# ohsnyt/bzip2-rust

Measured on AMD Instinct MI355X. Metric: compress MB/s at -9 (900 KB blocks), 1/2/4/8 MI355X; bit-exact vs C bzip2, higher is better.
Workload: dtype u8; 1 GPU; 1024 MiB per GPU synthetic text at -9 (1194 blocks on this rank), BASELINE configs[2]; raw_bytes_total=1073741824, blocks_rank0=1194, compressed_bytes=323302688

## Files before the change

### bzip2-rust_amd/csrc/bzx_bsort.hip

```cpp
#include <hip/hip_runtime.h>
#include "bzx_host.h"
#include "bzx_wg.h"
#include "bzx_pack.h"

#define BS_NT 1024
#define BS_NW (BS_NT / 64)
#ifndef BS_C
#define BS_C 2048
#endif
#define BS_FW (BS_C / 64)
#define BS_ISO (BS_C / 3)
#ifndef BS_ISO_SHIFT
#define BS_ISO_SHIFT 5
#endif
#ifndef BS_BIN1
#define BS_BIN1 15
#endif
#define BS_BIN2 12
#define BS_NBIN1 (1u << BS_BIN1)
#define BS_TAB_WORDS (BS_NBIN1 + (BS_NBIN1 >> 5))
#define BS_MAX_BK 1024
#ifndef BS_MAX_BIG
#define BS_MAX_BIG 512
#endif
// ... 190 lines not shown
    __syncthreads();
    return b_bcast[4] == 0;
}

struct BzxDeepItem {
    uint32_t blk, st, cnt, dbits;
};

__device__ __forceinline__ uint32_t *rank_array(const BzxBatch &B, uint32_t k, uint32_t which)
{
    if (k >= B.rk_blocks) return nullptr;
    return B.isa2 + ((size_t)k * 2 + which) * BZX_MAX_N;
}

__device__ __forceinline__ void emit_giant(const BzxBatch &B, uint32_t blk, uint64_t *rec_a, const uint64_t *rec_b,
                                           uint32_t st, uint32_t cnt, uint32_t depth, uint32_t bits)
{
    const uint32_t tid = threadIdx.x, base = st & 0x7fffffffu;
    const uint64_t *src = ((st >> 31) ? rec_b : rec_a) + base;
    uint32_t *__restrict__ isa0 = rank_array(B, (uint32_t)BZX_SLAB(B, blk), 0), *__restrict__ isa1 = rank_array(B, (uint32_t)BZX_SLAB(B, blk), 1);
    if (tid == 0) b_bcast[7] = isa0 ? atomicAdd(&B.counters[BZX_CTR_GIANT_CNT], 1u) : 0xFFFFFFFFu;
    __syncthreads();
    const uint32_t at = b_bcast[7];
    const bool listed = at < B.deep_cap;
    for (uint32_t i = tid; i < cnt; i += BS_NT) {
        const uint64_t r = src[i];
        rec_a[base + i] = (uint64_t)REC_IDX(r) | (i == 0 ? 1ull << 32 : 0ull);
        if (isa0) isa0[REC_IDX(r)] = isa1[REC_IDX(r)] = base | (listed ? 0u : RK_COARSE);
    }
    if (tid == 0) {
        atomicMin(&B.blk[blk].n_mtf, depth / bits);
        if (listed) {
            BzxDeepItem it;
            it.blk = blk;
            it.st = base;
            it.cnt = cnt;
            it.dbits = 0;
            reinterpret_cast<BzxDeepItem *>(B.deep_list)[(size_t)2 * B.deep_cap + at] = it;
        }
        atomicAdd(&B.blk[blk].n_groups, 1u);
        if ((atomicOr(&B.blk[blk].status, BZX_ST_RESUME) & BZX_ST_RESUME) == 0)
            B.resume_list[atomicAdd(&B.counters[BZX_CTR_RESUME], 1u)] = blk;
    }
    __syncthreads();
}

__device__ __forceinline__ void block_redo(const BzxBatch &B, uint32_t b)
{
    if ((atomicOr(&B.blk[b].status, BZX_ST_REDO) & BZX_ST_REDO) == 0)
        B.redo_list[atomicAdd(&B.counters[BZX_CTR_REDO], 1u)] = b;
}


__device__ bool deep_process(const BzxBatch &B, uint32_t b, uint32_t j_, uint32_t n, uint32_t bits, const uint8_t *__restrict__ P,
                             uint64_t *__restrict__ rec_a, uint64_t *__restrict__ rec_b, uint32_t done, uint32_t flush_from,
                             int push_lvl)
{
    const uint32_t tid = threadIdx.x;
    bool ok = true;
    while (ok) {
        const uint32_t nbig = b_bcast[3];
        __syncthreads();
        if (done >= nbig) break;
        if (push_lvl >= 0 && done >= flush_from) {
            const uint32_t np = nbig - done;
            if (tid == 0) b_bcast[5] = atomicAdd(&B.counters[BZX_CTR_DEEP_CNT + push_lvl], np);
            __syncthreads();
            const uint32_t at = b_bcast[5];
            __syncthreads();
            if (at + np <= B.deep_cap) {
                BzxDeepItem *dl = reinterpret_cast<BzxDeepItem *>(B.deep_list) + (size_t)(push_lvl & 1) * B.deep_cap + at;
                for (uint32_t q = tid; q < np; q += BS_NT) {
                    const uint32_t r = (done + q) % BS_MAX_BIG;
                    BzxDeepItem it;
                    it.blk = b;
                    it.st = b_big[r][0];
                    it.cnt = b_big[r][1];
                    it.dbits = b_big[r][2] | (bits << 16);
                    dl[q] = it;
                }
                __syncthreads();
                break;
            }
            push_lvl = -1;
        }
        const uint32_t st = b_big[done % BS_MAX_BIG][0], cnt = b_big[done % BS_MAX_BIG][1], depth = b_big[done % BS_MAX_BIG][2];
        done++;
        if (tid == 0) b_bcast[6] = atomicAdd(reinterpret_cast<uint32_t *>(&B.blk[b].pack_word), 1u);
        __syncthreads();
        const uint32_t spent = b_bcast[6];
        const uint32_t base = st & 0x7fffffffu, buf = st >> 31;
        const uint64_t *__restrict__ src = (buf ? rec_b : rec_a) + base;
        uint64_t *__restrict__ dst = (buf ? rec_a : rec_b) + base;
        if (depth + BS_BIN2 + 32 >= n * bits) {
            ok = false;
            break;
        }
        if (depth + BS_BIN2 > BS_MAX_DEPTH || spent >= BS_MAX_SPLITS) {
            emit_giant(B, b, rec_a, rec_b, st, cnt, depth, bits);
            continue;
        }
        constexpr uint32_t NB2 = 1u << BS_BIN2;
        for (uint32_t i = tid; i < NB2 + (NB2 >> 5); i += BS_NT) b_tab[i] = 0;
        if (tid == 0) b_bcast[1] = 0;
        if (tid < 3) b_bcast[8 + tid] = 0;
        __syncthreads();
        for (uint32_t i = tid; i < cnt; i += BS_NT) atomicAdd(&TAB((uint32_t)(src[i] >> (64 - BS_BIN2))), 1u);
// ... 96 lines not shown
                for (uint32_t e = 0; e < 4; e++)
                    if (i0 + e < n) atomicAdd(&TAB((uint32_t)((x[u] << (e * bits)) >> (64 - BS_BIN1))), 1u);
            }
        }
        __syncthreads();
        DIAG_STAMP(99);
        uint32_t nbk = form_buckets<(int)BS_NBIN1, true>(n);
        if (nbk) bucket_setup<BS_BIN1>(nbk);
        __syncthreads();
        DIAG_STAMP(100);
        if (nbk == 0) {
            DIAG_COUNT(106, 1);
            if (tid == 0) block_redo(B, b);
            __syncthreads();
            continue;
        }

        {
            constexpr uint32_t SP_TILE = 8192, SP_V = SP_TILE / (BS_NT * 4);
            static_assert(BS_MAX_BK <= BS_NT && BS_TAB_WORDS >= 32768 + BS_MAX_BK, "tile scan: one bucket per lane");
            uint16_t *tab16 = reinterpret_cast<uint16_t *>(b_tab);
            for (uint32_t i = tid; i < BS_NBIN1 / 2; i += BS_NT) {
                uint32_t v = reinterpret_cast<uint32_t *>(b_tab)[i];
                v |= ((uint32_t)b_b0[v & 1023u] << 10) | ((uint32_t)b_b0[(v >> 16) & 1023u] << 26);
                reinterpret_cast<uint32_t *>(b_tab)[i] = v;
            }
            uint64_t *stage = reinterpret_cast<uint64_t *>(b_tab + 16384);
            uint32_t *tcnt0 = b_tab + 32768;
            uint32_t *delta = b_first;
            uint32_t *tcnt1 = tcnt0 + BS_MAX_BK;
            if (tid < nbk) tcnt0[tid] = tcnt1[tid] = 0;
            uint64_t hi[SP_V], lo[SP_V];
            uint32_t pv[SP_V];
            auto load_tile = [&](uint32_t t0) {
#pragma unroll
                for (uint32_t u = 0; u < SP_V; u++) {
                    const uint32_t i0 = t0 + (u * BS_NT + tid) * 4;
                    hi[u] = lo[u] = 0;
                    pv[u] = 0;
                    if (i0 < n) {
                        uint64_t w2[2];
                        __builtin_memcpy(w2, P + ((i0 * bits) >> 3), 16);
                        hi[u] = w2[0];
                        lo[u] = w2[1];
                        if (i0 >= 1 && i0 + 3 <= n) {
                            __builtin_memcpy(&pv[u], T + i0 - 1, 4);
                        } else {
                            const uint32_t nvalid = n - i0 < 4u ? n - i0 : 4u;
                            for (uint32_t e = 0; e < nvalid; e++) pv[u] |= (uint32_t)T[i0 + e ? i0 + e - 1 : n - 1] << (8 * e);
                        }
                    }
                }
            };
            load_tile(0);
            bzx_lds_barrier();
            uint32_t tpar = 0;
            for (uint32_t t0 = 0; t0 < n; t0 += SP_TILE, tpar ^= 1u) {
                uint32_t *tcnt = tpar ? tcnt1 : tcnt0, *tother = tpar ? tcnt0 : tcnt1;
                uint32_t kr[SP_V * 4], key[SP_V * 4], pvc[SP_V];
#pragma unroll
                for (uint32_t u = 0; u < SP_V; u++) {
                    const uint32_t i0 = t0 + (u * BS_NT + tid) * 4;
                    const uint32_t nvalid = i0 < n ? (n - i0 < 4u ? n - i0 : 4u) : 0u;
                    const uint32_t sh0 = (i0 * bits) & 7u;
                    const uint64_t h = __builtin_bswap64(hi[u]), l = __builtin_bswap64(lo[u]);
                    pvc[u] = pv[u];
#pragma unroll
                    for (uint32_t e = 0; e < 4; e++) {
                        kr[u * 4 + e] = 0xFFFFFFFFu;
                        key[u * 4 + e] = 0;
                        if (e < nvalid) {
                            const uint32_t sh = sh0 + e * bits;
                            const uint64_t w = sh ? (h << sh) | (l >> (64u - sh)) : h;
                            const uint32_t kb = tab16[(uint32_t)(w >> (64 - BS_BIN1))], k = kb & 1023u;
                            key[u * 4 + e] = (uint32_t)((w << (kb >> 10)) >> 32);
                            kr[u * 4 + e] = k | (atomicAdd(&tcnt[k], 1u) << 16);
                        }
                    }
                }
                if (t0 + SP_TILE < n) load_tile(t0 + SP_TILE);
                bzx_lds_barrier();
                {
                    const uint32_t c = tid < nbk ? tcnt[tid] : 0u;
                    const uint32_t incl = bzx_wave_incl_sum(c);
                    uint32_t *wtot = b_scratch + tpar * BS_NW;
                    if (bzx_lane() == 63) wtot[bzx_wave()] = incl;
                    bzx_lds_barrier();
                    uint32_t pre = 0;
                    const uint32_t wv = bzx_wave();
#pragma unroll
                    for (uint32_t i = 0; i < BS_NW; i++) pre += i < wv ? wtot[i] : 0u;
                    const uint32_t ex = pre + incl - c;
                    if (tid < nbk) {
                        tcnt[tid] = ex;
                        tother[tid] = 0;
                        delta[tid] = b_start[tid] + b_cur[tid] - ex;
                        b_cur[tid] += c;
                    }
                }
                bzx_lds_barrier();
#pragma unroll
                for (uint32_t u = 0; u < SP_V; u++)
#pragma unroll
                    for (uint32_t e = 0; e < 4; e++)
                        if (kr[u * 4 + e] != 0xFFFFFFFFu) {
                            const uint32_t k = kr[u * 4 + e] & 0xFFFFu, rel = (u * BS_NT + tid) * 4 + e;
                            stage[tcnt[k] + (kr[u * 4 + e] >> 16)] = ((uint64_t)key[u * 4 + e] << 32) | ((uint64_t)k << 21) | ((uint64_t)rel << 8) |
                                                                     (uint64_t)((pvc[u] >> (8 * e)) & 255u);
                        }
                bzx_lds_barrier();
                const uint32_t tn = n - t0 < SP_TILE ? n - t0 : SP_TILE;
#pragma unroll
                for (uint32_t u = 0; u < SP_TILE / BS_NT; u++) {
                    const uint32_t i = u * BS_NT + tid;
                    if (i < tn) {
                        const uint64_t r = stage[i];
                        const uint32_t k = (uint32_t)(r >> 21) & 1023u, rel = (uint32_t)(r >> 8) & 8191u;
                        rec_a[delta[k] + i] = (r & 0xFFFFFFFF00000000ull) | ((uint64_t)(t0 + rel) << 12) | ((r & 255ull) << 4);
                    }
                }
            }
        }
        __syncthreads();
        DIAG_STAMP(101);
        bool ok = bucket_emit<BS_BIN1>(B, b, j_, nbk, 0, 0, 0, bits, 0, 0);
        DIAG_STAMP(102);

        if (ok) ok = deep_process(B, b, j_, n, bits, P, rec_a, rec_b, 0, 0, BZX_DEEP_LEVELS > 0 ? 0 : -1);
        DIAG_STAMP(103);
        if (!ok) DIAG_COUNT(107, 1);
        if (!ok && tid == 0) block_redo(B, b);
        __syncthreads();
    }
    DIAG_FLUSH();
}

__global__ __launch_bounds__(BS_NT) void bzx_bsplit_deep_kernel(BzxBatch B)
{
    const uint32_t tid = threadIdx.x, lvl = B.deep_lvl;
    const uint32_t listed = B.counters[BZX_CTR_DEEP_CNT + lvl];
    const uint32_t n_items = listed < B.deep_cap ? listed : B.deep_cap;
    if (n_items == 0) return;
    DIAG_T0();
    const BzxDeepItem *list = reinterpret_cast<const BzxDeepItem *>(B.deep_list) + (size_t)(lvl & 1u) * B.deep_cap;
    for (;;) {
        if (tid == 0) b_bcast[0] = atomicAdd(&B.counters[BZX_CTR_DEEP_FETCH + lvl], 1u);
        __syncthreads();
        const uint32_t i = b_bcast[0];
        __syncthreads();
        if (i >= n_items) break;
        const BzxDeepItem d = list[i];
        if (d.cnt == 0) continue;
        const uint32_t b = d.blk;
        if (__atomic_load_n(&B.blk[b].status, __ATOMIC_RELAXED) & BZX_ST_REDO) continue;
        const uint32_t n = B.blk[b].n, bits = d.dbits >> 16;
        const size_t sb = BZX_SLAB(B, b);
        const uint8_t *__restrict__ P = B.pk + sb * BZX_PK_STRIDE;
        uint64_t *__restrict__ rec_a = B.rec_a + sb * BZX_MAX_N;
        uint64_t *__restrict__ rec_b = B.rec_b + sb * BZX_MAX_N;
        if (tid == 0) {
            b_bcast[3] = 1;
            b_bcast[4] = 0;
            b_big[0][0] = d.st;
            b_big[0][1] = d.cnt;
            b_big[0][2] = d.dbits & 0xFFFFu;
        }
        __syncthreads();
        const bool ok = deep_process(B, b, (b - B.blk_first) / B.blk_step, n, bits, P, rec_a, rec_b, 0, 1,
                                     lvl + 1 < BZX_DEEP_LEVELS ? (int)lvl + 1 : -1);
        if (!ok && tid == 0) block_redo(B, b);
        __syncthreads();
    }
    DIAG_FLUSH();
}

#ifndef SK_NT
#define SK_NT 256
#endif
#define SK_NW (SK_NT / 64)
#define BS_E (BS_C / SK_NT)
#define SK_DB 8
#define SK_ND (1u << SK_DB)
static_assert(BS_C % SK_NT == 0 && BS_E >= 1 && BS_E <= 8, "bucket capacity");

__shared__ uint64_t s_x[BS_C];
__shared__ __attribute__((aligned(16))) uint64_t s_w[BS_C + 4];
__shared__ __attribute__((aligned(16))) uint32_t s_cnt[SK_NW][SK_ND];
__shared__ uint32_t s_dbase[SK_ND];
__shared__ uint32_t s_part[4];
__shared__ uint64_t s_f[BS_FW + 1];
__shared__ uint32_t s_med[BS_C / BS_TINY + 1];
__shared__ uint32_t s_large[BS_C / BS_MED + 1];
__shared__ uint32_t s_rc[2][4];
__shared__ uint32_t s_bc[8];
__shared__ uint32_t s_m[2];
__shared__ uint32_t s_red[SK_NW][4];

__device__ __forceinline__ uint32_t uni(uint32_t v) { return bzx_uni(v); }
__device__ __forceinline__ uint32_t tid_here() { return bzx_tid_here(); }
__device__ __forceinline__ BzxBucket uni(BzxBucket b)
{
    BzxBucket r;
    r.blk = uni(b.blk);
    r.start = uni(b.start);
    r.cnt = uni(b.cnt);
    if (r.cnt >> 31) r.cnt = 0;
    r.dbits = uni(b.dbits);
    return r;
}

__device__ __forceinline__ void wave_rank(uint32_t *wc, uint32_t d, bool valid, uint32_t lane, uint32_t &old, uint32_t &rank)
{
    uint64_t m = __ballot(valid);
    uint32_t plo = (uint32_t)m, phi = (uint32_t)(m >> 32);
#pragma unroll
    for (int b = 0; b < SK_DB; b++) {
        const uint32_t mask = 0u - ((d >> b) & 1u);
        m = __ballot((d >> b) & 1u);
        plo &= ~((uint32_t)m ^ mask);
        phi &= ~((uint32_t)(m >> 32) ^ mask);
    }
    const uint64_t peers = ((uint64_t)phi << 32) | plo;
    rank = (uint32_t)__popcll(peers & ((1ull << lane) - 1ull));
    old = wc[d];
    lds_order();
    if (valid && rank == 0) atomicAdd(&wc[d], (uint32_t)__popcll(peers));
    lds_order();
}

__device__ __attribute__((noinline)) void wg_radix_sort(uint32_t base, uint32_t cnt, int lo, int hi)
{
    uint64_t *A = s_w + base;
    const uint32_t tid = threadIdx.x, lane = bzx_lane(), wave = bzx_wave();
    const uint32_t rows = (cnt + SK_NT - 1) / SK_NT, chunk = rows * 64;
    if (tid == 0) {
// ... 95 lines not shown
            a1 &= s_red[w][3];
        }
        diff = ((uint64_t)(o1 & ~a1) << 32) | (o0 & ~a0);
    }
    uint32_t *wc = s_cnt[wave];
    uint32_t *wb = reinterpret_cast<uint32_t *>(s_w) + wave * SK_ND;
    for (int shift = lo; shift < hi; shift += SK_DB) {
        if (((diff >> shift) & (uint64_t)(SK_ND - 1)) == 0) continue;
#pragma unroll
        for (uint32_t i = 0; i < SK_ND / 64; i++) wc[i * 64 + lane] = 0;
        lds_order();
        uint64_t v[BS_E];
        uint32_t old[BS_E];
#pragma unroll
        for (uint32_t j = 0; j < BS_E; j++) {
            const uint32_t e = wave * chunk + j * 64 + lane;
            v[j] = j < rows && e < cnt ? A[e] : 0ull;
        }
#pragma unroll
        for (uint32_t j = 0; j < BS_E; j++) {
            const uint32_t e = wave * chunk + j * 64 + lane;
            old[j] = bzx_lds_ticket(&wc[(uint32_t)(v[j] >> shift) & (SK_ND - 1)], j < rows && e < cnt);
        }
        __syncthreads();
        {
            static_assert(SK_ND == 4 * 64, "four digits per lane");
            uint32_t mine[4], tot[4], sum = 0;
#pragma unroll
            for (uint32_t i = 0; i < 4; i++) mine[i] = tot[i] = 0;
#pragma unroll
            for (uint32_t w = 0; w < SK_NW; w++) {
                const uint4 c = *reinterpret_cast<const uint4 *>(&s_cnt[w][4 * lane]);
                const uint32_t cc[4] = {c.x, c.y, c.z, c.w};
#pragma unroll
                for (uint32_t i = 0; i < 4; i++) {
                    if (w < wave) mine[i] += cc[i];
                    tot[i] += cc[i];
                }
            }
#pragma unroll
            for (uint32_t i = 0; i < 4; i++) sum += tot[i];
            uint32_t run = bzx_wave_incl_sum(sum) - sum;
            uint4 o;
            o.x = run + mine[0];
            run += tot[0];
            o.y = run + mine[1];
            run += tot[1];
            o.z = run + mine[2];
            run += tot[2];
            o.w = run + mine[3];
            *reinterpret_cast<uint4 *>(&wb[4 * lane]) = o;
        }
        lds_order();
#pragma unroll
        for (uint32_t j = 0; j < BS_E; j++) {
            const uint32_t e = wave * chunk + j * 64 + lane;
            if (j < rows && e < cnt) A[wb[(uint32_t)(v[j] >> shift) & (SK_ND - 1)] + old[j]] = v[j];
        }
        __syncthreads();
    }
}

template <bool TICKETS>
__device__ __attribute__((noinline)) void wave_radix_sort(uint32_t base, uint32_t s, int lo, int hi)
{
    constexpr uint32_t ROWS = BS_MED / 64;
    uint64_t *A = s_w + base;
    uint32_t *wc = s_cnt[bzx_wave()];
    const uint32_t lane = bzx_lane();
    const uint32_t rows = (s + 63u) / 64u;
    uint64_t v[ROWS];
    uint64_t diff = 0;
    {
        const uint64_t a0 = A[0];
#pragma unroll
        for (uint32_t j = 0; j < ROWS; j++) {
            const uint32_t e = j * 64 + lane;
            v[j] = e < s ? A[e] : 0ull;
            if (e < s) diff |= v[j] ^ a0;
        }
#pragma unroll
        for (int sh = 32; sh > 0; sh >>= 1) diff |= __shfl_xor(diff, sh);
    }
    for (int shift = lo; shift < hi; shift += SK_DB) {
        if (((diff >> shift) & (uint64_t)(SK_ND - 1)) == 0) continue;
#pragma unroll
        for (uint32_t i = 0; i < SK_ND / 64; i++) wc[i * 64 + lane] = 0;
        lds_order();
        uint32_t old[ROWS], rk[ROWS];
#pragma unroll
        for (uint32_t j = 0; j < ROWS; j++) {
            old[j] = rk[j] = 0;
            if (j < rows) {
                if (TICKETS) old[j] = bzx_lds_ticket(&wc[(uint32_t)(v[j] >> shift) & (SK_ND - 1)], j * 64 + lane < s);
                else wave_rank(wc, (uint32_t)(v[j] >> shift) & (SK_ND - 1), j * 64 + lane < s, lane, old[j], rk[j]);
            }
        }
        {
            uint32_t c[SK_ND / 64], sum = 0;
#pragma unroll
            for (uint32_t i = 0; i < SK_ND / 64; i++) {
                c[i] = wc[(SK_ND / 64) * lane + i];
                sum += c[i];
            }
            uint32_t run = bzx_wave_incl_sum(sum) - sum;
            lds_order();
#pragma unroll
            for (uint32_t i = 0; i < SK_ND / 64; i++) {
                wc[(SK_ND / 64) * lane + i] = run;
                run += c[i];
            }
        }
        lds_order();
#pragma unroll
        for (uint32_t j = 0; j < ROWS; j++)
            if (j * 64 + lane < s) A[wc[(uint32_t)(v[j] >> shift) & (SK_ND - 1)] + old[j] + rk[j]] = v[j];
        lds_order();
#pragma unroll
        for (uint32_t j = 0; j < ROWS; j++) {
            const uint32_t e = j * 64 + lane;
            v[j] = e < s ? A[e] : 0ull;
        }
        lds_order();
    }
}

__device__ __forceinline__ uint32_t fbit(uint32_t p) { return (uint32_t)(s_f[p >> 6] >> (p & 63u)) & 1u; }
__device__ __forceinline__ void fset(uint32_t p) { atomicOr((unsigned long long *)&s_f[p >> 6], 1ull << (p & 63u)); }

__device__ __forceinline__ bool tiny_bounds(uint32_t p, uint32_t &gs, uint32_t &ge)
{
    const uint32_t wi = p >> 6, bi = p & 63u;
    uint64_t w = s_f[wi] & (~0ull >> (63u - bi));
    if (w) {
        gs = wi * 64 + 63u - (uint32_t)__builtin_clzll(w);
    } else {
        if (wi == 0) return false;
        w = s_f[wi - 1];
        if (!w) return false;
        gs = (wi - 1) * 64 + 63u - (uint32_t)__builtin_clzll(w);
    }
    w = bi == 63u ? 0ull : s_f[wi] & (~0ull << (bi + 1u));
    if (w) {
        ge = wi * 64 + (uint32_t)__builtin_ctzll(w);
    } else {
        w = s_f[wi + 1];
        if (!w) return false;
        ge = (wi + 1) * 64 + (uint32_t)__builtin_ctzll(w);
    }
    return ge - gs <= BS_TINY;
}

__device__ __forceinline__ void mark_changes(uint32_t base, uint32_t s, int lo, uint32_t t, uint32_t step)
{
    for (uint32_t e = 1 + t; e < s; e += step)
        if ((s_w[base + e] >> lo) != (s_w[base + e - 1] >> lo)) fset(base + e);
}

__device__ __forceinline__ bool any_big(uint32_t base, uint32_t s, uint32_t t, uint32_t step)
{
    bool big = false;
    for (uint32_t e = t; e < s; e += step) {
        uint32_t gs, ge;
        big |= !tiny_bounds(base + e, gs, ge);
    }
    return big;
}

__device__ __forceinline__ void wave_sort_mark(uint32_t base, uint32_t s, int lo, uint32_t lane)
// ... 93 lines not shown
        wg_radix_sort(gs, sz, 48, 64);
        mark_changes(gs, sz, 48, tid, SK_NT);
        if (tid == 0) s_bc[2] = 0;
        __syncthreads();
        if (any_big(gs, sz, tid, SK_NT)) s_bc[2] = 1;
        __syncthreads();
        if (s_bc[2]) {
            wg_radix_sort(gs, sz, 14, 64);
            mark_changes(gs, sz, 14, tid, SK_NT);
        }
    }
    __syncthreads();
}

template <typename RankOf>
__device__ __forceinline__ void rank_tiny_groups(uint32_t amask, uint32_t nrow, const RankOf &rank_of, uint32_t (&dst_)[BS_E],
                                                 uint64_t (&my)[BS_E])
{
#pragma unroll
    for (uint32_t j = 0; j < BS_E; j++) {
        dst_[j] = 0xFFFFFFFFu;
        my[j] = 0;
        uint32_t a_ = 0, sz = 0;
        if ((amask >> j) & 1u) {
            const uint32_t p = rank_of(j);
            uint32_t e_;
            if (tiny_bounds(p, a_, e_) && e_ - a_ > 1) {
                sz = e_ - a_;
                my[j] = s_w[p];
            }
        }
        if (j < nrow) {
            uint32_t r = 0, rk = 0;
            const uint64_t myc = my[j] & ~W_POS_MASK;
            for (uint32_t i = 0; i < sz; i += 4) {
                uint64_t wq[4];
#pragma unroll
                for (uint32_t k = 0; k < 4; k++) wq[k] = s_w[a_ + i + k];
#pragma unroll
                for (uint32_t k = 0; k < 4; k++) {
                    const bool in = i + k < sz;
                    r += in && wq[k] < my[j];
                    rk += in && wq[k] < myc;
                }
            }
            if (sz) dst_[j] = (a_ + r) | (r != rk ? 0u : 0x80000000u);
        }
    }
    __syncthreads();
}

__device__ __forceinline__ void place_ranked(const uint32_t (&dst_)[BS_E], const uint64_t (&my)[BS_E])
{
#pragma unroll
    for (uint32_t j = 0; j < BS_E; j++) {
        if (dst_[j] != 0xFFFFFFFFu) {
            const uint32_t q = dst_[j] & 0x7FFFFFFFu;
            s_w[q] = my[j];
            if ((dst_[j] >> 31) && !fbit(q)) fset(q);
        }
    }
    __syncthreads();
}

#define LIST(which, i) (reinterpret_cast<uint16_t *>(s_x)[4u * (i) + 2u + (which)])

template <bool ALL>
__device__ __attribute__((noinline)) void list_tied(uint32_t n, uint32_t from, uint32_t to)
{
    const uint32_t tid = tid_here(), lane = tid & 63u;
    const uint32_t nrow = (n + SK_NT - 1) / SK_NT;
#pragma unroll
    for (uint32_t j = 0; j < BS_E; j++) {
        if (j < nrow) {
            const uint32_t i = j * SK_NT + tid;
            uint32_t p = 0;
            bool t = false;
            if (i < n) {
                p = ALL ? i : (uint32_t)LIST(from, i);
                t = !(fbit(p) && fbit(p + 1));
            }
            const uint64_t mk = __ballot(t);
            if (mk) {
                uint32_t base = 0;
                if (lane == 0) base = atomicAdd(&s_m[to], (uint32_t)__popcll(mk));
                base = bzx_bcast0(base);
                if (t) LIST(to, base + (uint32_t)__popcll(mk & ((1ull << lane) - 1ull))) = (uint16_t)p;
            }
        }
    }
}

__device__ __forceinline__ bool initial_sort(uint32_t cnt)
{
    const uint32_t tid = tid_here(), lane = tid & 63u, wave = tid >> 6;
    uint64_t fm[BS_E];
    wg_radix_sort_opt(cnt, 64 - BS_KEYBITS, 64);
    int bad = 0;
#pragma unroll
    for (uint32_t j = 0; j < BS_E; j++) {
        const uint32_t p = j * SK_NT + tid;
        s_w[p] = p;
        const uint64_t kp = s_x[p] >> (64 - BS_KEYBITS), kq = p ? s_x[p - 1] >> (64 - BS_KEYBITS) : 0ull;
        const bool f = p >= cnt || p == 0 || kp != kq;
        bad |= p < cnt && p > 0 && kp < kq;
        fm[j] = __ballot(f);
        if (lane == 0) s_f[j * SK_NW + wave] = fm[j];
    }
    if (tid == 0) s_f[BS_FW] = ~0ull;
    if (__syncthreads_or(bad)) return false;
#pragma unroll
    for (uint32_t j = 0; j < BS_E; j++) {
// ... 140 lines not shown
        }
        if (tid < 4) s_rc[0][tid] = 0;
        if (tid < 2) s_m[tid] = 0;
        DIAG_STAMP(65);
        if (!initial_sort(cnt)) {
            if (tid == 0) {
                atomicAdd(&B.counters[BZX_CTR_STAT0 + 15], 1u);
                block_redo(B, b);
            }
            PREFETCH_NEXT();
            __syncthreads();
            it = nit;
            nit = uni(nit2);
            n_cur = uni(n_nx);
            st_cur = uni(st_nx);
            continue;
        }
        DIAG_STAMP(67);

        uint32_t dcur = depth0 + BS_KEYBITS;
        bool fail = false;
        uint32_t lpar = 0;
        __syncthreads();
        DIAG_STAMP(73);
        for (uint32_t round = 0;; round++) {
            tid = tid_here();
            lane = tid & 63u;
            wave = tid >> 6;
            const uint32_t par = round & 1u;
            const uint32_t m = uni(s_m[lpar]);
            if (m == 0) break;
            if (m <= 64) {
                DIAG_COUNT(89, 1);
                if (wave == 0) {
                    dcur = wave_rounds(P, bits, nbits, m, lpar, round, dcur);
                    if (lane == 0) s_bc[3] = dcur;
                }
                __syncthreads();
                dcur = uni(s_bc[3]);
                fail = dcur >> 31;
                dcur &= 0x7FFFFFFFu;
                DIAG_STAMP(70);
                break;
            }
            if (!(round < BS_ROUNDS && dcur < nbits)) {
                DIAG_COUNT(round >= BS_ROUNDS ? 84 : 85, 1);
                fail = true;
                break;
            }
            DIAG_COUNT(80, 1);
            DIAG_COUNT(88, m);
            const uint32_t nrow = (m + SK_NT - 1) / SK_NT;
            uint32_t amask = 0, hmask = 0;
            uint32_t pq[BS_E], xa[BS_E];
#pragma unroll
            for (uint32_t j = 0; j < BS_E; j++) {
                pq[j] = 0;
                xa[j] = 0;
                if (j < nrow) {
                    const uint32_t i = j * SK_NT + tid;
                    if (i < m) {
                        const uint32_t p = LIST(lpar, i);
                        amask |= 1u << j;
                        hmask |= fbit(p) << j;
                        pq[j] = p | ((uint32_t)(s_w[p] & W_POS_MASK) << 16);
                    }
                }
            }
#pragma unroll
            for (uint32_t j = 0; j < BS_E; j++) {
                if ((amask >> j) & 1u) {
                    uint32_t x = REC_IDX(s_x[pq[j] >> 16]) * bits + dcur;
                    if (x >= nbits) x -= nbits;
                    xa[j] = x;
                }
            }
            uint64_t g[BS_E];
#pragma unroll
            for (uint32_t j = 0; j < BS_E; j++) g[j] = ((amask >> j) & 1u) ? pk_window_bit(P, xa[j]) : 0ull;
            const auto rank_of = [&](uint32_t j) { return pq[j] & 0xFFFFu; };
            list_big_groups(hmask, par, rank_of);
#pragma unroll
            for (uint32_t j = 0; j < BS_E; j++)
                if ((amask >> j) & 1u) s_w[pq[j] & 0xFFFFu] = (g[j] & ~W_POS_MASK) | (uint64_t)(pq[j] >> 16);
            if (tid == 0) {
                s_rc[par ^ 1u][0] = s_rc[par ^ 1u][1] = s_rc[par ^ 1u][2] = s_rc[par ^ 1u][3] = 0;
                s_m[lpar ^ 1u] = 0;
            }
            __syncthreads();
            DIAG_STAMP(68);
            const uint32_t nmed = s_rc[par][1], nlarge = s_rc[par][2];
            if (nmed | nlarge) {
                DIAG_COUNT(86, nmed);
                DIAG_COUNT(87, nlarge);
                sort_listed_groups(par, nmed, nlarge, tid, lane);
                DIAG_STAMP(69);
            }
            tid = tid_here();
            lane = tid & 63u;
            wave = tid >> 6;
            uint32_t dst_[BS_E];
            uint64_t my[BS_E];
            rank_tiny_groups(amask, nrow, rank_of, dst_, my);
            DIAG_STAMP(70);
            place_ranked(dst_, my);
            DIAG_STAMP(71);
            list_tied<false>(m, lpar, lpar ^ 1u);
            __syncthreads();
            DIAG_STAMP(73);
            lpar ^= 1u;
            dcur += 50;
        }
        PREFETCH_NEXT();
        tid = tid_here();
        if (fail || B.bsort_mode == 1) {
            uint64_t *__restrict__ sax = B.rec_a + BZX_SLAB(B, b) * BZX_MAX_N + start;
            const uint32_t rk = uni(B.blk[b].n_selectors);
            uint32_t *__restrict__ isa0 = rank_array(B, rk, 0), *__restrict__ isa1 = rank_array(B, rk, 1);
#pragma unroll
            for (uint32_t j = 0; j < BS_E; j++) {
                const uint32_t p = j * SK_NT + tid;
                if (p < cnt) {
                    const uint32_t rot = REC_IDX(s_x[(uint32_t)(s_w[p] & W_POS_MASK)]);
                    const uint32_t f0 = fbit(p);
                    sax[p] = (uint64_t)rot | ((uint64_t)f0 << 32);
                    if (isa0) {
                        const uint32_t head = f0 ? p : group_start(p);
                        isa0[rot] = start + head;
                        if (f0 && fbit(p + 1)) isa1[rot] = start + head;
                    }
                }
            }
            if (fail) {
                uint32_t *__restrict__ cl = reinterpret_cast<uint32_t *>(B.rec_b + BZX_SLAB(B, b) * BZX_MAX_N + start);
                uint64_t mk[BS_E];
                lane = tid & 63u;
                wave = tid >> 6;
#pragma unroll
                for (uint32_t j = 0; j < BS_E; j++) mk[j] = tied_mask(s_f[j * SK_NW + wave], s_f[j * SK_NW + wave + 1]);
                slot_counts_publish(mk, BS_E);
                __syncthreads();
                uint32_t before[BS_E];
                const uint32_t total = slot_counts_sum(BS_E, before);
#pragma unroll
                for (uint32_t j = 0; j < BS_E; j++) {
                    if ((mk[j] >> lane) & 1ull) {
                        const uint32_t p = j * SK_NT + tid;
                        const uint32_t rot = REC_IDX(s_x[(uint32_t)(s_w[p] & W_POS_MASK)]);
                        cl[before[j] + (uint32_t)__popcll(mk[j] & ((1ull << lane) - 1ull))] = p | (fbit(p) << 11) | (rot << 12);
                    }
                }
                if (tid == 0) {
                    atomicMin(&B.blk[b].n_mtf, dcur / bits);
                    B.bk_list[idx].cnt = cnt | 0x80000000u;
                    const uint32_t ri = atomicAdd(&B.counters[BZX_CTR_RK_ITEMS], 1u);
                    B.rk_list[ri] = idx;
                    B.rk_list[B.bk_cap + ri] = total;
                    atomicAdd(&B.counters[BZX_CTR_RK_OPEN], 1u);
                    atomicAdd(&B.blk[b].n_groups, 1u);
                    if ((atomicOr(&B.blk[b].status, BZX_ST_RESUME) & BZX_ST_RESUME) == 0)
                        B.resume_list[atomicAdd(&B.counters[BZX_CTR_RESUME], 1u)] = b;
                }
            }
        }
        {
            constexpr uint32_t OUT_E = 8;
            uint8_t *__restrict__ L = B.bwt + BZX_SLAB(B, b) * BZX_BLK_STRIDE + start;
            const uint32_t p0 = tid * OUT_E;
            if (p0 < cnt) {
                const uint32_t rot = tid >> 2;
                uint32_t pos[OUT_E];
#pragma unroll
                for (uint32_t k = 0; k < OUT_E; k++) pos[k] = (uint32_t)(s_w[p0 + ((k + rot) & (OUT_E - 1))] & W_POS_MASK);
                uint64_t bytes = 0;
#pragma unroll
                for (uint32_t k = 0; k < OUT_E; k++) {
                    const uint32_t kk = (k + rot) & (OUT_E - 1);
                    const uint32_t r = reinterpret_cast<const uint32_t *>(s_x)[2u * pos[k]];
                    bytes |= (uint64_t)REC_PREV(r) << (8 * kk);
                    if (p0 + kk < cnt && REC_IDX(r) == 0) B.blk[b].orig_ptr = start + p0 + kk;
                }
                if (p0 + OUT_E <= cnt) {
                    __builtin_memcpy(L + p0, &bytes, 8);
                } else {
                    for (uint32_t k = 0; p0 + k < cnt; k++) L[p0 + k] = (uint8_t)(bytes >> (8 * k));
                }
            }
            DIAG_COUNT(83, 1);
        }
        __syncthreads();
        DIAG_STAMP(72);
        it = nit;
        nit = uni(nit2);
        n_cur = uni(n_nx);
        st_cur = uni(st_nx);
    }
    DIAG_FLUSH();
}

__global__ __launch_bounds__(SK_NT, SK_WAVES_PER_SIMD) void bzx_bsort_kernel(BzxBatch B) { bsort_body(B); }
__global__ __launch_bounds__(SK_NT, SK_WAVES_PER_SIMD) void bzx_bfill_kernel(BzxBatch B) { bsort_body(B); }

#define RK_CHUNK 16
struct RkMeta {
    uint32_t bi, T, blk, start, cnt, n, rk, h0;
};
__shared__ RkMeta s_meta[RK_CHUNK];

__device__ __forceinline__ uint32_t rk_fetch_chunk(const BzxBatch &B, uint32_t n_items, uint32_t &open)
{
    __shared__ uint32_t s_fetch[2];
    __syncthreads();
    if (threadIdx.x < 64) {
        uint32_t base = 0;
        if (threadIdx.x == 0) base = atomicAdd(&B.counters[B.rk_fetch], (uint32_t)RK_CHUNK);
        base = __shfl(base, 0);
        const uint32_t i = base + threadIdx.x;
        bool op = false;
        if (threadIdx.x < RK_CHUNK && i < n_items) {
            RkMeta m;
            m.bi = B.rk_list[i];
            m.T = B.rk_list[B.bk_cap + i];
            const BzxBucket it = B.bk_list[m.bi];
            op = !(it.dbits >> 31);
            m.blk = it.blk;
            m.start = it.start & 0x7fffffffu;
            m.cnt = it.cnt & 0x7fffffffu;
            m.n = B.blk[it.blk].n;
            m.rk = B.blk[it.blk].n_selectors;
            m.h0 = B.blk[it.blk].n_mtf;
            s_meta[threadIdx.x] = m;
        }
        const uint64_t m = __ballot(op);
        if (threadIdx.x == 0) {
// ... 558 lines not shown
```

### bzip2-rust_amd/csrc/bzx_wg.h

```cpp
#pragma once
#include <hip/hip_runtime.h>
#include <stdint.h>

#define BZX_WAVE 64

#ifdef BZX_HIP_EMU
#define bzx_lds_barrier() __syncthreads()
#else
#define bzx_lds_barrier() asm volatile("s_waitcnt lgkmcnt(0)\n\ts_barrier" ::: "memory")
#endif

#ifdef BZX_HIP_EMU
#define bzx_wave_sync() hipemu::wave_sync()
#else
#define bzx_wave_sync()                                      \
    do {                                                     \
        __builtin_amdgcn_fence(__ATOMIC_SEQ_CST, "wavefront"); \
        __builtin_amdgcn_wave_barrier();                     \
    } while (0)
#endif


#ifdef BZX_HIP_EMU
__device__ inline uint32_t bzx_lds_ticket(uint32_t *ctr, bool valid)
{
    static uintptr_t who[16][64];
    const uint32_t lane = threadIdx.x & 63u, wave = threadIdx.x >> 6;
    const uintptr_t me = valid ? (uintptr_t)ctr : 0;
    who[wave][lane] = me;
    hipemu::wave_sync();
    uint32_t before = 0, same = 0;
    for (uint32_t l = 0; l < 64; l++) {
        if (valid && who[wave][l] == me) {
            same++;
            if (l < lane) before++;
        }
    }
    const uint32_t base = valid ? *ctr : 0u;
    hipemu::wave_sync();
    if (valid && before == 0) *ctr = base + same;
    hipemu::wave_sync();
    return base + before;
}
#else
__device__ __forceinline__ uint32_t bzx_lds_ticket(uint32_t *ctr, bool valid) { return valid ? atomicAdd(ctr, 1u) : 0u; }
#endif
#ifdef BZX_HIP_EMU
#define lds_order() hipemu::wave_sync()
__device__ __forceinline__ uint32_t bzx_uni(uint32_t v) { return v; }
__device__ __forceinline__ uint32_t bzx_bcast0(uint32_t v) { return __shfl(v, 0); }
__device__ __forceinline__ uint32_t bzx_tid_here() { return threadIdx.x; }
#define bzx_drain_stores() do {} while (0)
#else
#define lds_order() asm volatile("" ::: "memory")
__device__ __forceinline__ uint32_t bzx_uni(uint32_t v) { return (uint32_t)__builtin_amdgcn_readfirstlane((int)v); }
__device__ __forceinline__ uint32_t bzx_bcast0(uint32_t v) { return (uint32_t)__builtin_amdgcn_readfirstlane((int)v); }
__device__ __forceinline__ uint32_t bzx_tid_here()
{
    uint32_t t = threadIdx.x;
    asm volatile("" : "+v"(t));
    return t;
}
#define bzx_drain_stores() asm volatile("s_waitcnt vmcnt(0)" ::: "memory")
#endif

#ifdef BZX_HIP_EMU
#define BZX_HOST_PORTABLE 0u
#define BZX_MBUF_CHUNK_MIN ((size_t)64 << 10)
#else
#define BZX_HOST_PORTABLE hipHostMallocPortable
#define BZX_MBUF_CHUNK_MIN ((size_t)16 << 20)
#endif

#ifdef BZX_HIP_EMU
__device__ inline uint32_t bzx_lane_prev(uint32_t v)
{
    const uint32_t y = __shfl_up(v, 1);
    return (threadIdx.x & 63u) ? y : 0u;
}
#else
__device__ __forceinline__ uint32_t bzx_lane_prev(uint32_t v)
{
    return (uint32_t)__builtin_amdgcn_update_dpp(0, (int)v, 0x138, 0xf, 0xf, false);
}
#endif

__device__ __forceinline__ uint32_t bzx_lane() { return threadIdx.x & 63u; }
__device__ __forceinline__ uint32_t bzx_wave() { return threadIdx.x >> 6; }

__device__ __forceinline__ uint64_t bzx_match_any(uint32_t d, int nbits, bool valid)
{
    uint64_t peers = __ballot(valid);
    for (int b = 0; b < nbits; b++) {
        const bool bit = (d >> b) & 1u;
        const uint64_t m = __ballot(bit);
        peers &= bit ? m : ~m;
    }
    return peers;
}

#ifdef BZX_HIP_EMU
#define BZX_DPP_SCAN(v, OP, IDENT)                                           \
    do {                                                                     \
        const uint32_t lane_ = bzx_lane();                                   \
        for (uint32_t d_ = 1; d_ < 64; d_ <<= 1) {                           \
            const uint32_t y_ = __shfl_up(v, d_);                            \
// ... 161 lines not shown
```

Measured before the change: 29650 MB/s.

## Batch LDS loads ahead of dependent stores across bucket-sort kernels

Restructures several hot loops in the block-sort kernels so independent LDS and global loads are issued as a batch before their dependent atomics and stores. It adds a full-tile fast path in the initial split, hoists scatter addresses and flag-word loads, processes the refine loop in groups of up to four rows, and adds an asm register barrier (bzx_landed) to force loads to complete before use. The aim is more memory-level parallelism and fewer serialized LDS round trips. In exchange it raises register pressure, which can lower occupancy, and duplicates code paths.

```diff
diff --git a/bzip2-rust_amd/csrc/bzx_bsort.hip b/bzip2-rust_amd/csrc/bzx_bsort.hip
--- a/bzip2-rust_amd/csrc/bzx_bsort.hip
+++ b/bzip2-rust_amd/csrc/bzx_bsort.hip
@@ -266,7 +266,7 @@
 }
 
 
-__device__ bool deep_process(const BzxBatch &B, uint32_t b, uint32_t j_, uint32_t n, uint32_t bits, const uint8_t *__restrict__ P,
+__device__ __forceinline__ bool deep_process(const BzxBatch &B, uint32_t b, uint32_t j_, uint32_t n, uint32_t bits, const uint8_t *__restrict__ P,
                              uint64_t *__restrict__ rec_a, uint64_t *__restrict__ rec_b, uint32_t done, uint32_t flush_from,
                              int push_lvl)
 {
@@ -469,12 +469,48 @@
                     }
                 }
             };
+            auto window_landed = [&]() {
+#pragma unroll
+                for (uint32_t u = 0; u < SP_V; u++) {
+                    bzx_landed(hi[u]);
+                    bzx_landed(lo[u]);
+                    bzx_landed(pv[u]);
+                }
+            };
             load_tile(0);
+            window_landed();
             bzx_lds_barrier();
             uint32_t tpar = 0;
-            for (uint32_t t0 = 0; t0 < n; t0 += SP_TILE, tpar ^= 1u) {
+            const uint32_t ns = bzx_uni(n);
+            for (uint32_t t0 = 0; t0 < ns; t0 += SP_TILE, tpar ^= 1u) {
                 uint32_t *tcnt = tpar ? tcnt1 : tcnt0, *tother = tpar ? tcnt0 : tcnt1;
                 uint32_t kr[SP_V * 4], key[SP_V * 4], pvc[SP_V];
+                const bool full = t0 + SP_TILE <= ns;
+                if (full) {
+                    uint64_t w[SP_V * 4];
+                    uint32_t kb[SP_V * 4];
+#pragma unroll
+                    for (uint32_t u = 0; u < SP_V; u++) {
+                        const uint32_t i0 = t0 + (u * BS_NT + tid) * 4;
+                        const uint32_t sh0 = (i0 * bits) & 7u;
+                        const uint64_t h = __builtin_bswap64(hi[u]), l = __builtin_bswap64(lo[u]);
+                        pvc[u] = pv[u];
+#pragma unroll
+                        for (uint32_t e = 0; e < 4; e++) {
+                            const uint32_t sh = sh0 + e * bits;
+                            w[u * 4 + e] = sh ? (h << sh) | (l >> (64u - sh)) : h;
+                        }
+                    }
+#pragma unroll
+                    for (uint32_t q = 0; q < SP_V * 4; q++) kb[q] = tab16[(uint32_t)(w[q] >> (64 - BS_BIN1))];
+#pragma unroll
+                    for (uint32_t q = 0; q < SP_V * 4; q++) kr[q] = atomicAdd(&tcnt[kb[q] & 1023u], 1u);
+#pragma unroll
+                    for (uint32_t q = 0; q < SP_V * 4; q++) {
+                        key[q] = (uint32_t)((w[q] << (kb[q] >> 10)) >> 32);
+                        kr[q] = (kb[q] & 1023u) | (kr[q] << 16);
+                    }
+                } else {
 #pragma unroll
                 for (uint32_t u = 0; u < SP_V; u++) {
                     const uint32_t i0 = t0 + (u * BS_NT + tid) * 4;
@@ -495,6 +531,7 @@
                         }
                     }
                 }
+                }
                 if (t0 + SP_TILE < n) load_tile(t0 + SP_TILE);
                 bzx_lds_barrier();
                 {
@@ -516,6 +553,19 @@
                     }
                 }
                 bzx_lds_barrier();
+                if (full) {
+                    uint32_t tb[SP_V * 4];
+#pragma unroll
+                    for (uint32_t q = 0; q < SP_V * 4; q++) tb[q] = tcnt[kr[q] & 0xFFFFu];
+#pragma unroll
+                    for (uint32_t u = 0; u < SP_V; u++)
+#pragma unroll
+                        for (uint32_t e = 0; e < 4; e++) {
+                            const uint32_t q = u * 4 + e, k = kr[q] & 0xFFFFu, rel = (u * BS_NT + tid) * 4 + e;
+                            stage[tb[q] + (kr[q] >> 16)] = ((uint64_t)key[q] << 32) | ((uint64_t)k << 21) | ((uint64_t)rel << 8) |
+                                                           (uint64_t)((pvc[u] >> (8 * e)) & 255u);
+                        }
+                } else {
 #pragma unroll
                 for (uint32_t u = 0; u < SP_V; u++)
 #pragma unroll
@@ -525,8 +575,23 @@
                             stage[tcnt[k] + (kr[u * 4 + e] >> 16)] = ((uint64_t)key[u * 4 + e] << 32) | ((uint64_t)k << 21) | ((uint64_t)rel << 8) |
                                                                      (uint64_t)((pvc[u] >> (8 * e)) & 255u);
                         }
+                }
                 bzx_lds_barrier();
+                window_landed();
                 const uint32_t tn = n - t0 < SP_TILE ? n - t0 : SP_TILE;
+                if (full) {
+                    uint64_t r[SP_TILE / BS_NT];
+                    uint32_t dl[SP_TILE / BS_NT];
+#pragma unroll
+                    for (uint32_t u = 0; u < SP_TILE / BS_NT; u++) r[u] = stage[u * BS_NT + tid];
+#pragma unroll
+                    for (uint32_t u = 0; u < SP_TILE / BS_NT; u++) dl[u] = delta[(uint32_t)(r[u] >> 21) & 1023u];
+#pragma unroll
+                    for (uint32_t u = 0; u < SP_TILE / BS_NT; u++) {
+                        const uint32_t rel = (uint32_t)(r[u] >> 8) & 8191u;
+                        rec_a[dl[u] + u * BS_NT + tid] = (r[u] & 0xFFFFFFFF00000000ull) | ((uint64_t)(t0 + rel) << 12) | ((r[u] & 255ull) << 4);
+                    }
+                } else {
 #pragma unroll
                 for (uint32_t u = 0; u < SP_TILE / BS_NT; u++) {
                     const uint32_t i = u * BS_NT + tid;
@@ -535,6 +600,7 @@
                         const uint32_t k = (uint32_t)(r >> 21) & 1023u, rel = (uint32_t)(r >> 8) & 8191u;
                         rec_a[delta[k] + i] = (r & 0xFFFFFFFF00000000ull) | ((uint64_t)(t0 + rel) << 12) | ((r & 255ull) << 4);
                     }
+                }
                 }
             }
         }
@@ -598,6 +664,7 @@
 #define BS_E (BS_C / SK_NT)
 #define SK_DB 8
 #define SK_ND (1u << SK_DB)
+#define BS_G (BS_E < 4 ? BS_E : 4)
 static_assert(BS_C % SK_NT == 0 && BS_E >= 1 && BS_E <= 8, "bucket capacity");
 
 __shared__ uint64_t s_x[BS_C];
@@ -799,10 +866,15 @@
             *reinterpret_cast<uint4 *>(&wb[4 * lane]) = o;
         }
         lds_order();
+        uint32_t at[BS_E];
+#pragma unroll
+        for (uint32_t j = 0; j < BS_E; j++) at[j] = wb[(uint32_t)(v[j] >> shift) & (SK_ND - 1)] + old[j];
+#pragma unroll
+        for (uint32_t j = 0; j < BS_E; j++) bzx_landed(at[j]);
 #pragma unroll
         for (uint32_t j = 0; j < BS_E; j++) {
             const uint32_t e = wave * chunk + j * 64 + lane;
-            if (j < rows && e < cnt) A[wb[(uint32_t)(v[j] >> shift) & (SK_ND - 1)] + old[j]] = v[j];
+            if (j < rows && e < cnt) A[at[j]] = v[j];
         }
         __syncthreads();
     }
@@ -838,10 +910,8 @@
 #pragma unroll
         for (uint32_t j = 0; j < ROWS; j++) {
             old[j] = rk[j] = 0;
-            if (j < rows) {
-                if (TICKETS) old[j] = bzx_lds_ticket(&wc[(uint32_t)(v[j] >> shift) & (SK_ND - 1)], j * 64 + lane < s);
-                else wave_rank(wc, (uint32_t)(v[j] >> shift) & (SK_ND - 1), j * 64 + lane < s, lane, old[j], rk[j]);
-            }
+            if (TICKETS) old[j] = bzx_lds_ticket(&wc[(uint32_t)(v[j] >> shift) & (SK_ND - 1)], j * 64 + lane < s);
+            else if (j < rows) wave_rank(wc, (uint32_t)(v[j] >> shift) & (SK_ND - 1), j * 64 + lane < s, lane, old[j], rk[j]);
         }
         {
             uint32_t c[SK_ND / 64], sum = 0;
@@ -859,9 +929,14 @@
             }
         }
         lds_order();
+        uint32_t at[ROWS];
+#pragma unroll
+        for (uint32_t j = 0; j < ROWS; j++) at[j] = wc[(uint32_t)(v[j] >> shift) & (SK_ND - 1)] + old[j] + rk[j];
+#pragma unroll
+        for (uint32_t j = 0; j < ROWS; j++) bzx_landed(at[j]);
 #pragma unroll
         for (uint32_t j = 0; j < ROWS; j++)
-            if (j * 64 + lane < s) A[wc[(uint32_t)(v[j] >> shift) & (SK_ND - 1)] + old[j] + rk[j]] = v[j];
+            if (j * 64 + lane < s) A[at[j]] = v[j];
         lds_order();
 #pragma unroll
         for (uint32_t j = 0; j < ROWS; j++) {
@@ -1061,12 +1136,15 @@
 
 __device__ __forceinline__ void place_ranked(const uint32_t (&dst_)[BS_E], const uint64_t (&my)[BS_E])
 {
+    uint64_t fw[BS_E];
+#pragma unroll
+    for (uint32_t j = 0; j < BS_E; j++) fw[j] = s_f[dst_[j] != 0xFFFFFFFFu ? (dst_[j] & 0x7FFFFFFFu) >> 6 : 0u];
 #pragma unroll
     for (uint32_t j = 0; j < BS_E; j++) {
         if (dst_[j] != 0xFFFFFFFFu) {
             const uint32_t q = dst_[j] & 0x7FFFFFFFu;
             s_w[q] = my[j];
-            if ((dst_[j] >> 31) && !fbit(q)) fset(q);
+            if ((dst_[j] >> 31) && !((fw[j] >> (q & 63u)) & 1ull)) fset(q);
         }
     }
     __syncthreads();
@@ -1313,37 +1391,48 @@
             DIAG_COUNT(88, m);
             const uint32_t nrow = (m + SK_NT - 1) / SK_NT;
             uint32_t amask = 0, hmask = 0;
-            uint32_t pq[BS_E], xa[BS_E];
-#pragma unroll
-            for (uint32_t j = 0; j < BS_E; j++) {
-                pq[j] = 0;
-                xa[j] = 0;
-                if (j < nrow) {
-                    const uint32_t i = j * SK_NT + tid;
-                    if (i < m) {
-                        const uint32_t p = LIST(lpar, i);
-                        amask |= 1u << j;
-                        hmask |= fbit(p) << j;
-                        pq[j] = p | ((uint32_t)(s_w[p] & W_POS_MASK) << 16);
-                    }
-                }
-            }
-#pragma unroll
-            for (uint32_t j = 0; j < BS_E; j++) {
-                if ((amask >> j) & 1u) {
-                    uint32_t x = REC_IDX(s_x[pq[j] >> 16]) * bits + dcur;
+            uint32_t pq[BS_E];
+            const auto rank_of = [&](uint32_t j) { return pq[j] & 0xFFFFu; };
+#pragma unroll
+            for (uint32_t j = 0; j < BS_E; j++) pq[j] = 0;
+#pragma unroll
+            for (uint32_t h0 = 0; h0 < BS_E; h0 += BS_G) {
+                if (h0 >= nrow) break;
+                uint32_t fl[BS_G], xa[BS_G];
+#pragma unroll
+                for (uint32_t k = 0; k < BS_G; k++) {
+                    const uint32_t j = h0 + k, i = j * SK_NT + tid;
+                    const bool has = j < nrow && i < m;
+                    amask |= (uint32_t)has << j;
+                    pq[j] = LIST(lpar, has ? i : 0u);
+                }
+#pragma unroll
+                for (uint32_t k = 0; k < BS_G; k++) {
+                    fl[k] = reinterpret_cast<const uint32_t *>(s_f)[pq[h0 + k] >> 5];
+                    xa[k] = reinterpret_cast<const uint32_t *>(s_w)[2u * pq[h0 + k]];
+                }
+#pragma unroll
+                for (uint32_t k = 0; k < BS_G; k++) {
+                    const uint32_t j = h0 + k;
+                    hmask |= (((fl[k] >> (pq[j] & 31u)) & 1u) & (amask >> j)) << j;
+                    pq[j] |= (xa[k] & (uint32_t)W_POS_MASK) << 16;
+                }
+#pragma unroll
+                for (uint32_t k = 0; k < BS_G; k++) xa[k] = reinterpret_cast<const uint32_t *>(s_x)[2u * (pq[h0 + k] >> 16)];
+#pragma unroll
+                for (uint32_t k = 0; k < BS_G; k++) {
+                    uint32_t x = REC_IDX(xa[k]) * bits + dcur;
                     if (x >= nbits) x -= nbits;
-                    xa[j] = x;
-                }
-            }
-            uint64_t g[BS_E];
-#pragma unroll
-            for (uint32_t j = 0; j < BS_E; j++) g[j] = ((amask >> j) & 1u) ? pk_window_bit(P, xa[j]) : 0ull;
-            const auto rank_of = [&](uint32_t j) { return pq[j] & 0xFFFFu; };
-            list_big_groups(hmask, par, rank_of);
-#pragma unroll
-            for (uint32_t j = 0; j < BS_E; j++)
-                if ((amask >> j) & 1u) s_w[pq[j] & 0xFFFFu] = (g[j] & ~W_POS_MASK) | (uint64_t)(pq[j] >> 16);
+                    xa[k] = ((amask >> (h0 + k)) & 1u) ? x : 0u;
+                }
+                uint64_t g[BS_G];
+#pragma unroll
+                for (uint32_t k = 0; k < BS_G; k++) g[k] = pk_window_bit(P, xa[k]);
+                list_big_groups(hmask & (((1u << BS_G) - 1u) << h0), par, rank_of);
+#pragma unroll
+                for (uint32_t k = 0; k < BS_G; k++)
+                    if ((amask >> (h0 + k)) & 1u) s_w[pq[h0 + k] & 0xFFFFu] = (g[k] & ~W_POS_MASK) | (uint64_t)(pq[h0 + k] >> 16);
+            }
             if (tid == 0) {
                 s_rc[par ^ 1u][0] = s_rc[par ^ 1u][1] = s_rc[par ^ 1u][2] = s_rc[par ^ 1u][3] = 0;
                 s_m[lpar ^ 1u] = 0;
@@ -1433,14 +1522,18 @@
                 uint32_t pos[OUT_E];
 #pragma unroll
                 for (uint32_t k = 0; k < OUT_E; k++) pos[k] = (uint32_t)(s_w[p0 + ((k + rot) & (OUT_E - 1))] & W_POS_MASK);
+                uint32_t r[OUT_E];
+#pragma unroll
+                for (uint32_t k = 0; k < OUT_E; k++) r[k] = reinterpret_cast<const uint32_t *>(s_x)[2u * pos[k]];
                 uint64_t bytes = 0;
+                uint32_t row0 = 0xFFFFFFFFu;
 #pragma unroll
                 for (uint32_t k = 0; k < OUT_E; k++) {
                     const uint32_t kk = (k + rot) & (OUT_E - 1);
-                    const uint32_t r = reinterpret_cast<const uint32_t *>(s_x)[2u * pos[k]];
-                    bytes |= (uint64_t)REC_PREV(r) << (8 * kk);
-                    if (p0 + kk < cnt && REC_IDX(r) == 0) B.blk[b].orig_ptr = start + p0 + kk;
-                }
+                    bytes |= (uint64_t)REC_PREV(r[k]) << (8 * kk);
+                    if (p0 + kk < cnt && REC_IDX(r[k]) == 0) row0 = start + p0 + kk;
+                }
+                if (row0 != 0xFFFFFFFFu) B.blk[b].orig_ptr = row0;
                 if (p0 + OUT_E <= cnt) {
                     __builtin_memcpy(L + p0, &bytes, 8);
                 } else {
diff --git a/bzip2-rust_amd/csrc/bzx_wg.h b/bzip2-rust_amd/csrc/bzx_wg.h
--- a/bzip2-rust_amd/csrc/bzx_wg.h
+++ b/bzip2-rust_amd/csrc/bzx_wg.h
@@ -51,7 +51,9 @@
 __device__ __forceinline__ uint32_t bzx_bcast0(uint32_t v) { return __shfl(v, 0); }
 __device__ __forceinline__ uint32_t bzx_tid_here() { return threadIdx.x; }
 #define bzx_drain_stores() do {} while (0)
-#else
+#define bzx_landed(x) do {} while (0)
+#else
+#define bzx_landed(x) asm volatile("" : "+v"(x))
 #define lds_order() asm volatile("" ::: "memory")
 __device__ __forceinline__ uint32_t bzx_uni(uint32_t v) { return (uint32_t)__builtin_amdgcn_readfirstlane((int)v); }
 __device__ __forceinline__ uint32_t bzx_bcast0(uint32_t v) { return (uint32_t)__builtin_amdgcn_readfirstlane((int)v); }
```

New measurement: 29850 MB/s (median of 6 runs). Within noise of the previous version (+0.7%).
